# HagenMarin/SHAP-Transformer-ASR

Measured on NVIDIA B200. Metric: masked_coalition_forwards_per_sec, higher is better.
Workload: dtype bf16

## Files before the change

### include/w2s.h

```cpp
#ifndef W2S_H_
#define W2S_H_

#include <stdint.h>

#ifdef __cplusplus
extern "C" {
#endif

typedef struct w2s_handle w2s_handle;

#define W2S_MAX_CONV_LAYERS 8

enum {
  W2S_OUT_MAX     = 0,
  W2S_OUT_LOGIT   = 1,
  W2S_OUT_LOGPROB = 2,
  W2S_OUT_MEAN    = 3,
  W2S_OUT_LOGITS  = 4,
  W2S_OUT_CTC     = 5
};

enum {
  W2S_FLAG_VALIDATE_GEMM = 1,
  W2S_FLAG_VALIDATE_ATTN = 2,
// ... 63 lines not shown

int w2s_grad_waveforms(w2s_handle* h, const float* x_dev, int64_t n, int64_t L, int64_t ld,
                       const int32_t* frames_host, float* grad_dev, float* out_dev, void* stream);
int w2s_vjp_waveforms(w2s_handle* h, const float* x_dev, int64_t n, int64_t L, int64_t ld, const float* gout_dev,
                      float* grad_dev, float* out_dev, void* stream);
int w2s_grad_transcripts(w2s_handle* h, const float* x_dev, int64_t n, int64_t L, int64_t ld, const int32_t* which_host,
                         float* grad_dev, float* out_dev, void* stream);
int w2s_grad_debug(w2s_handle* h, int on);
int w2s_grad_rules(w2s_handle* h, int rules);
int64_t w2s_grad_peek(w2s_handle* h, const char* name, void* dst_dev, int64_t max_bytes, void* stream);

int w2s_mask(w2s_handle* h, const uint32_t* z_bits_dev, int64_t K, float* out_dev, void* stream);

int w2s_wls(w2s_handle* h, const uint32_t* z_bits_dev, const double* w_dev, const float* y_dev, int64_t K,
            int M, int D, const double* fx_dev, const double* fnull_dev, double* phi_dev, int32_t* status_dev,
            void* stream);

int64_t w2s_sample_rows(int M, int n_full, int n_paired, const int64_t* ind_set, int64_t n_ind,
                        int64_t samples_left, int64_t added, uint32_t* mt_key, int32_t* mt_pos,
                        uint32_t* z_words, double* weights, int64_t cap_rows, int64_t* ind_used);

int w2s_relative_buckets(int T, int num_buckets, int max_distance, int32_t* out);

int w2s_debug_gemm(int use_tcgen05, const void* a_bf16, const void* w_bf16, const float* bias,
                   const void* residual, int res_fp32, float alpha, void* out, int M, int N, int K, int act,
                   int out_fp32, void* stream);
int w2s_debug_attention(int use_tcgen05, const void* qkv, const void* pos_proj, int B, int T, int heads, float scale,
                        void* ctx, float* lse, void* stream);
int w2s_debug_attention_bias(int use_tcgen05, const void* qkv, const float* rel_bias, const float* gate, int B, int T,
                             int heads, float scale, void* ctx, float* lse, void* stream);
int w2s_debug_attention_bwd(int use_tcgen05, const void* qkv, const void* ctx, const void* dctx, const float* lse, int B,
                            int T, int heads, float scale, void* dqkv, void* stream);
int w2s_debug_ctc(const float* logits, int n, int T, int V, int ldl, const int32_t* labels_host, const int32_t* offsets_host,
                  int D, int blank, const int32_t* which_host, float* out_dev, float* dlogits_dev, void* stream);
int w2s_profile_enable(w2s_handle* h, int on);
int64_t w2s_profile_read(w2s_handle* h, char* names, int64_t names_cap, double* ms, double* flops, double* bytes,
                         int64_t* counts, int64_t max_entries);
int w2s_kernel_count(const w2s_handle* h, int64_t* launches_per_batch, int64_t* batch_tile);
int64_t w2s_launch_count(const w2s_handle* h);
double w2s_flops_per_forward(const w2s_handle* h, int64_t num_samples);

#ifdef __cplusplus
}
#endif
#endif
```

### shap_transformer_asr_b200/_lib.py

```python
from __future__ import annotations

import ctypes as C
import os

_HERE = os.path.dirname(os.path.abspath(__file__))
LIB_PATH = os.path.join(_HERE, "libw2s.so")

MAX_CONV_LAYERS = 8

OUT_MAX, OUT_LOGIT, OUT_LOGPROB, OUT_MEAN, OUT_LOGITS, OUT_CTC = 0, 1, 2, 3, 4, 5
MODE_IDS = {"max": OUT_MAX, "logit": OUT_LOGIT, "logprob": OUT_LOGPROB, "mean": OUT_MEAN, "logits": OUT_LOGITS}
FLAG_VALIDATE_GEMM, FLAG_VALIDATE_ATTN, FLAG_FP32_PRELN, FLAG_NO_GRAPH = 1, 2, 4, 16
MAX_BACKGROUND = 256
MAX_BANDS = 16
MAX_TRANSCRIPT = 512


class W2SConfig(C.Structure):
    _fields_ = [
        ("kind", C.c_int32),
        ("num_conv_layers", C.c_int32),
        ("conv_dim", C.c_int32 * MAX_CONV_LAYERS),
        ("conv_kernel", C.c_int32 * MAX_CONV_LAYERS),
        ("conv_stride", C.c_int32 * MAX_CONV_LAYERS),
# ... 35 lines not shown
    "w2s_set_transcripts": (C.c_int, [C.c_void_p, C.POINTER(C.c_int32), C.POINTER(C.c_int32), C.c_int, C.c_int,
                                      C.c_void_p]),
    "w2s_out_width": (C.c_int64, [C.c_void_p, C.c_int64]),
    "w2s_eval": (C.c_int, [C.c_void_p, C.c_void_p, C.c_int64, C.c_void_p, C.c_void_p]),
    "w2s_eval_waveforms": (C.c_int, [C.c_void_p, C.c_void_p, C.c_int64, C.c_int64, C.c_int64, C.c_void_p,
                                     C.c_void_p]),
    "w2s_grad_waveforms": (C.c_int, [C.c_void_p, C.c_void_p, C.c_int64, C.c_int64, C.c_int64, C.POINTER(C.c_int32),
                                     C.c_void_p, C.c_void_p, C.c_void_p]),
    "w2s_vjp_waveforms": (C.c_int, [C.c_void_p, C.c_void_p, C.c_int64, C.c_int64, C.c_int64, C.c_void_p, C.c_void_p,
                                    C.c_void_p, C.c_void_p]),
    "w2s_grad_transcripts": (C.c_int, [C.c_void_p, C.c_void_p, C.c_int64, C.c_int64, C.c_int64, C.POINTER(C.c_int32),
                                       C.c_void_p, C.c_void_p, C.c_void_p]),
    "w2s_grad_debug": (C.c_int, [C.c_void_p, C.c_int]),
    "w2s_grad_rules": (C.c_int, [C.c_void_p, C.c_int]),
    "w2s_grad_peek": (C.c_int64, [C.c_void_p, C.c_char_p, C.c_void_p, C.c_int64, C.c_void_p]),
    "w2s_mask": (C.c_int, [C.c_void_p, C.c_void_p, C.c_int64, C.c_void_p, C.c_void_p]),
    "w2s_wls": (C.c_int, [C.c_void_p, C.c_void_p, C.c_void_p, C.c_void_p, C.c_int64, C.c_int, C.c_int, C.c_void_p,
                          C.c_void_p, C.c_void_p, C.c_void_p, C.c_void_p]),
    "w2s_sample_rows": (C.c_int64, [C.c_int, C.c_int, C.c_int, C.c_void_p, C.c_int64, C.c_int64, C.c_int64, C.c_void_p,
                                    C.c_void_p, C.c_void_p, C.c_void_p, C.c_int64, C.c_void_p]),
    "w2s_relative_buckets": (C.c_int, [C.c_int, C.c_int, C.c_int, C.c_void_p]),
    "w2s_debug_gemm": (C.c_int, [C.c_int, C.c_void_p, C.c_void_p, C.c_void_p, C.c_void_p, C.c_int, C.c_float,
                                 C.c_void_p, C.c_int, C.c_int, C.c_int, C.c_int, C.c_int, C.c_void_p]),
    "w2s_debug_attention": (C.c_int, [C.c_int, C.c_void_p, C.c_void_p, C.c_int, C.c_int, C.c_int, C.c_float, C.c_void_p,
                                      C.c_void_p, C.c_void_p]),
    "w2s_debug_attention_bias": (C.c_int, [C.c_int, C.c_void_p, C.c_void_p, C.c_void_p, C.c_int, C.c_int, C.c_int, C.c_float,
                                           C.c_void_p, C.c_void_p, C.c_void_p]),
    "w2s_debug_attention_bwd": (C.c_int, [C.c_int, C.c_void_p, C.c_void_p, C.c_void_p, C.c_void_p, C.c_int, C.c_int, C.c_int,
                                          C.c_float, C.c_void_p, C.c_void_p]),
    "w2s_debug_ctc": (C.c_int, [C.c_void_p, C.c_int, C.c_int, C.c_int, C.c_int, C.POINTER(C.c_int32), C.POINTER(C.c_int32),
                                C.c_int, C.c_int, C.POINTER(C.c_int32), C.c_void_p, C.c_void_p, C.c_void_p]),
    "w2s_profile_enable": (C.c_int, [C.c_void_p, C.c_int]),
    "w2s_profile_read": (C.c_int64, [C.c_void_p, C.c_char_p, C.c_int64, C.POINTER(C.c_double), C.POINTER(C.c_double),
                                     C.POINTER(C.c_double), C.POINTER(C.c_int64), C.c_int64]),
    "w2s_kernel_count": (C.c_int, [C.c_void_p, C.POINTER(C.c_int64), C.POINTER(C.c_int64)]),
    "w2s_launch_count": (C.c_int64, [C.c_void_p]),
    "w2s_flops_per_forward": (C.c_double, [C.c_void_p, C.c_int64]),
}

_lib = None


def load():
    global _lib
    if _lib is not None:
        return _lib
# ... 12 lines not shown
```

### shap_transformer_asr_b200/csrc/api.cu

```cuda
#include "../../include/w2s.h"
#include "gemm.cuh"
#include "kernels.cuh"
#include "ctc.cuh"

#include <algorithm>
#include <cmath>
#include <cstdlib>
#include <cstring>
#include <functional>
#include <map>
#include <memory>
#include <string>
#include <vector>

using namespace w2s;
typedef __nv_bfloat16 bf16;

namespace {

thread_local std::string g_create_error;

struct LayerW {
  bf16 *wqkv = nullptr, *wo = nullptr, *w1 = nullptr, *w2 = nullptr;
  float *bqkv = nullptr, *bo = nullptr, *b1 = nullptr, *b2 = nullptr;
// ... 7 lines not shown
  float *gate_w = nullptr, *gate_b = nullptr, *gate_c = nullptr;
};

struct Step {
  std::string name;
  std::function<std::string(cudaStream_t)> run;
  double flops = 0.0;
  double bytes = 0.0;
};

struct ProfRec {
  std::string name;
  cudaEvent_t e0, e1;
  double flops, bytes;
};

struct Plan {
  int n = 0;
  std::vector<Step> steps;
  std::vector<GemmLaunch*> gemms;
  std::vector<AttnRelPlan*> attn_rel;
  std::vector<PosConvPlan*> posconv;
  std::vector<AttnFaPlan*> attn_fa;
  cudaGraphExec_t exec = nullptr;
  bool graph_failed = false;
  ~Plan() {
    if (exec) cudaGraphExecDestroy(exec);
    for (auto* f : attn_fa) attention_fa_free(f);
    for (auto* pc : posconv) posconv_free(pc);
    for (auto* g : gemms) delete g;
    for (auto* a : attn_rel) attention_rel_free(a);
  }
};

__global__ void set_dyn_kernel(DynArgs* dst, const DynArgs v) { *dst = v; }

struct GradW {
  bf16 *wqkvT = nullptr, *woT = nullptr, *w1T = nullptr, *w2T = nullptr;
  bf16 *f2w1T = nullptr, *f2w2T = nullptr, *pw1T = nullptr, *pw2T = nullptr, *wqkT = nullptr, *wvT = nullptr;
  float* dw_flip = nullptr;
  bf16 *pos_proj = nullptr, *pos_projT = nullptr;
};
struct GradPlan;

}

struct w2s_handle {
  w2s_config cfg{};
  int device = 0;
  int num_sms = 148;
  bool auto_batch = false;
// ... 355 lines not shown
  W2S_CUDA_OK(cudaDeviceSynchronize());
  return "";
}

GemmProblem plain_problem(const bf16* a, long long rows, int K, const bf16* w, int N) {
  GemmProblem p;
  p.a = a; p.a_cols = K; p.a_rows = rows; p.a_batches = 1; p.a_row_stride = K; p.a_batch_stride = rows * (long long)K;
  p.a_kb_per_row = K / 64; p.a_g_col = 0;
  p.w = w; p.M = (int)rows; p.N = N; p.K = K; p.Bz = 1; p.G = 1;
  p.epi.ldg = 0; p.epi.ldb = 0; p.epi.ldm = N;
  return p;
}

int64_t num_frames(const w2s_config& c, int64_t L, std::vector<int>* lens) {
  int64_t n = L;
  for (int l = 0; l < c.num_conv_layers; ++l) {
    if (n < c.conv_kernel[l]) return 0;
    n = (n - c.conv_kernel[l]) / c.conv_stride[l] + 1;
    if (lens) lens->push_back((int)n);
  }
  return n;
}

void free_workspace(w2s_handle* h) {
  h->plans.clear();
  for (void* p : h->ws_allocs) cudaFree(p);
  h->ws_allocs.clear();
  h->ws_L = -1;
}

std::string ensure_workspace(w2s_handle* h, long long L) {
  if (h->ws_L == L) return "";
  cudaDeviceSynchronize();
  free_workspace(h);
  const w2s_config& c = h->cfg;
  h->Tl.clear();
  const int64_t T = num_frames(c, L, &h->Tl);
  if (T <= 0) return "clip of " + std::to_string(L) + " samples is shorter than the conv receptive field";
  h->T = (int)T;
  h->Tp = (int)((T + 63) / 64 * 64);
  if (h->auto_batch) {
    long long k = 1;
    while ((long long)h->num_sms * 128 * k / T < 128) ++k;
    long long tile = (long long)h->num_sms * 128 * k / T;
    const long long conv0_bytes = (long long)h->Tl[0] * c.conv_dim[0] * 2;
    while (tile > 8 && tile * conv0_bytes > (8LL << 30)) tile /= 2;
    h->cfg.max_batch = (int)tile;
  }
  const size_t nb = (size_t)c.max_batch;
  const int H = c.hidden_size, I = c.intermediate_size;
  const int Cl = c.conv_dim[c.num_conv_layers - 1];
  auto& pool = h->ws_allocs;
  W2S_TRY(dalloc(pool, &h->gn_a, nb * c.conv_dim[0]));
  W2S_TRY(dalloc(pool, &h->gn_b, nb * c.conv_dim[0]));
  W2S_TRY(dalloc(pool, &h->gn_wb, nb * c.conv_dim[0] * 32));
  size_t szA = 0, szB = 0;
  for (int l = 0; l < c.num_conv_layers; ++l) {
    const size_t s = nb * (size_t)h->Tl[l] * c.conv_dim[l];
    if (l % 2 == 0) szA = s > szA ? s : szA;
    else szB = s > szB ? s : szB;
  }
  W2S_TRY(dalloc(pool, &h->bufA, szA));
  W2S_TRY(dalloc(pool, &h->bufB, szB ? szB : 1));
  const size_t rows = nb * (size_t)T;
  W2S_TRY(dalloc(pool, &h->fpn, rows * Cl));
  W2S_TRY(dalloc(pool, &h->h0, rows * H));
  W2S_TRY(dalloc(pool, &h->hb, rows * H));
  W2S_TRY(dalloc(pool, &h->h1, rows * H));
  W2S_TRY(dalloc(pool, &h->pre, rows * H));
  W2S_TRY(dalloc(pool, &h->qkv, rows * 4 * H));
  W2S_TRY(dalloc(pool, &h->ctx, rows * H));
  W2S_TRY(dalloc(pool, &h->ffn, rows * I));
  W2S_TRY(dalloc(pool, &h->logits, rows * (size_t)h->head_ldl));
  if (c.kind != 1) {
    W2S_TRY(dalloc(pool, &h->hp,
                   nb * (size_t)(T + c.num_conv_pos_embeddings) * c.num_conv_pos_embedding_groups * 64));
    if (c.kind == 2) {
      const int heads = c.num_attention_heads;
      std::vector<int32_t> bk((size_t)(2 * T - 1));
      if (w2s_relative_buckets((int)T, c.num_buckets, c.max_bucket_distance, bk.data()) != 0)
// ... 70 lines not shown
    const int T = h->T, H = c.hidden_size, V = c.vocab_size;
    HeadParams hp{};
    hp.h = h->hb; hp.w = h->head_w; hp.bias = h->head_b;
    hp.n = n; hp.T = T; hp.H = H; hp.V = V; hp.ldl = h->head_ldl; hp.dyn = h->dyn_dev;
    if (simt_gemm) {
      add("head", [=](cudaStream_t s) { return launch_head(hp, s); });
      return "";
    }
    GemmProblem p = plain(h->hb, (long long)n * T, H, h->head_w, h->head_ldl);
    p.epi.bias = h->head_b;
    p.epi.out = h->logits;
    p.epi.out_fp32 = 1;
    W2S_TRY(add_gemm("lm_head", p));
    const float* logits = h->logits;
    add("head_reduce", [=](cudaStream_t s) { return launch_head_reduce(logits, hp, s); }, 0.0,
        (double)n * T * V * 4.0);
    return "";
  }

  std::string build() {
    const w2s_config& c = h->cfg;
    const int T = h->T, H = c.hidden_size, I = c.intermediate_size;
    const bool layer = c.feat_extract_norm == 1;
    const long long rows = (long long)n * T;
    w2s_handle* hh = h;
    const int nn = n;

    {
      Conv0Params cp{};
      cp.dyn = h->dyn_dev;
      cp.n = n; cp.L = (int)h->ws_L; cp.T0 = h->Tl[0]; cp.C = c.conv_dim[0]; cp.kw = c.conv_kernel[0];
      cp.stride = c.conv_stride[0];
      cp.w = h->conv0_w; cp.bias = h->conv0_b; cp.gamma = h->norm0_g; cp.beta = h->norm0_b;
      cp.gn_a = h->gn_a; cp.gn_b = h->gn_b; cp.gn_wb = h->gn_wb;
      cp.ln_wbar = h->ln0_wbar; cp.ln_gram = h->ln0_gram; cp.ln_wb = h->ln0_wb;
      cp.ln_bmean = h->ln0_bmean; cp.ln_b2mean = h->ln0_b2mean; cp.ln_wb48 = h->ln0_wb48;
      cp.out = h->bufA;
      const int fill = this->fill;
      const double wave_bytes = (fill == FILL_BANDS ? 4.0 * h->bands_F : fill == FILL_BG ? 8.0 : 4.0) * (double)h->ws_L;
      if (!layer)
        add("conv0_stats", [=](cudaStream_t s) { return launch_conv0_stats(cp, s, fill); }, 0.0,
            (wave_bytes + (double)cp.C * (8.0 + 64.0)) * n);
      add("conv0", [=](cudaStream_t s) { return launch_conv0(cp, layer, s, fill); },
          2.0 * cp.T0 * (double)cp.C * cp.kw * n, ((double)cp.T0 * cp.C * 2.0 + wave_bytes) * n);
    }
    bf16* cur = h->bufA;
    for (int l = 1; l < c.num_conv_layers; ++l) {
      bf16* nxt = (l % 2 == 1) ? h->bufB : h->bufA;
      const int Cin = c.conv_dim[l - 1], Cout = c.conv_dim[l], kw = c.conv_kernel[l], st = c.conv_stride[l];
      const int Tin = h->Tl[l - 1], Tout = h->Tl[l];
      if ((st * Cin) % 64) return "conv layer " + std::to_string(l) + ": stride * in_channels must be a multiple of 64";
      GemmProblem p;
      p.a = cur; p.a_cols = (long long)st * Cin; p.a_rows = (Tin + st - 1) / st; p.a_batches = n;
      p.a_row_stride = (long long)st * Cin; p.a_batch_stride = (long long)Tin * Cin;
      p.a_kb_per_row = st * Cin / 64; p.a_g_col = 0;
      p.w = h->conv_w[l]; p.M = Tout; p.N = Cout; p.K = kw * Cin; p.Bz = n; p.G = 1;
      p.epi.bias = h->conv_b[l];
      p.epi.act = layer ? ACT_NONE : ACT_GELU;
      p.epi.out = nxt; p.epi.ldb = (long long)Tout * Cout; p.epi.ldm = Cout;
      W2S_TRY(add_gemm("conv" + std::to_string(l), p));
      if (layer)
        add_ln("conv" + std::to_string(l) + "_ln_gelu", nxt, 0, (long long)n * Tout, Cout, h->conv_ln_g[l],
               h->conv_ln_b[l], 1e-5f, ACT_GELU, nxt, nullptr);
      cur = nxt;
    }
    const int Cl = c.conv_dim[c.num_conv_layers - 1];
    add_ln("featproj_ln", cur, 0, rows, Cl, h->fp_ln_g, h->fp_ln_b, c.layer_norm_eps, ACT_NONE, h->fpn, nullptr);
    {
      GemmProblem p = plain(h->fpn, rows, Cl, h->fp_w, H);
      p.epi.bias = h->fp_b;
// ... 841 lines not shown
                             h->wls_work, (cudaStream_t)stream);
  return e.empty() ? 0 : fail(h, e);
}

int w2s_debug_gemm(int use_tcgen05, const void* a_bf16, const void* w_bf16, const float* bias, const void* residual,
                   int res_fp32, float alpha, void* out, int M, int N, int K, int act, int out_fp32, void* stream) {
  g_create_error.clear();
  std::string e = gemm_init();
  if (e.empty()) {
    GemmProblem p = PlanBuilder::plain((const bf16*)a_bf16, M, K, (const bf16*)w_bf16, N);
    p.epi.bias = bias; p.epi.act = act; p.epi.out = out; p.epi.out_fp32 = out_fp32;
    p.epi.residual = residual; p.epi.res_fp32 = res_fp32; p.epi.alpha = alpha;
    GemmLaunch gl;
    e = gemm_prepare(p, debug_num_sms(), &gl);
    if (e.empty()) e = use_tcgen05 ? gemm_launch_tc(gl, (cudaStream_t)stream) : gemm_launch_simt(gl, (cudaStream_t)stream);
  }
  if (!e.empty()) {
    g_create_error = e;
    return 1;
  }
  return 0;
}

int w2s_debug_attention(int use_tcgen05, const void* qkv, const void* pos_proj, int B, int T, int heads, float scale,
                        void* ctx, float* lse, void* stream) {
  g_create_error.clear();
  const cudaStream_t s = (cudaStream_t)stream;
  AttnParams ap = debug_attn_params(qkv, pos_proj, B, T, heads, scale);
  ap.ctx = (bf16*)ctx;
  ap.lse = lse;
  std::string e;
  if (B <= 0 || T <= 0 || heads <= 0 || !qkv || !ctx) {
    e = "debug_attention: need B, T', heads >= 1 and qkv / ctx buffers";
  } else if (lse && (pos_proj || !use_tcgen05)) {
    e = "debug_attention: only the tcgen05 kernel without relative positions writes the log-sum-exp";
  } else if (!(e = gemm_init()).empty()) {
  } else if (!use_tcgen05) {
    e = launch_attention_simt(ap, s);
  } else if (pos_proj) {
    AttnRelPlan* rp = nullptr;
    e = attention_rel_init();
    if (e.empty()) e = attention_rel_prepare(ap, &rp);
    if (e.empty()) e = attention_rel_launch(rp, s);
    if (rp) attention_rel_free(rp);
  } else {
    AttnFaPlan* fp = nullptr;
// ... 234 lines not shown
```

### shap_transformer_asr_b200/csrc/frontend.cu

```cuda
#include "kernels.cuh"

namespace w2s {

template <int FILL>
__global__ void __launch_bounds__(256) mask_kernel(const float* __restrict__ x, const uint16_t* __restrict__ seg_id,
                                                    const uint32_t* __restrict__ zbits, int zwords, long long L,
                                                    float baseline, float* __restrict__ out, long long ld,
                                                    const float* __restrict__ bg, int B, long long bg_ld, long long row0) {
  constexpr bool BG = FILL == FILL_BG;
  __shared__ uint32_t z[64];
  const long long g = BG ? row0 + blockIdx.y : blockIdx.y;
  const long long k = BG ? g / B : g;
  if (threadIdx.x < zwords) z[threadIdx.x] = zbits[k * zwords + threadIdx.x];
  __syncthreads();
  const long long i0 = ((long long)blockIdx.x * blockDim.x + threadIdx.x) * 4;
  if (i0 >= L) return;
  float* o = out + g * ld + i0;
  if constexpr (FILL == FILL_BANDS) {
    const int F = B;
    auto keep = [&](uint32_t sgm, int b) { const uint32_t c = sgm * F + b; return (z[c >> 5] >> (c & 31)) & 1u; };
    if (i0 + 4 <= L && ((ld & 3) == 0) && (bg_ld & 3) == 0) {
      const ushort4 sv = *reinterpret_cast<const ushort4*>(seg_id + i0);
      float4 r = make_float4(0.f, 0.f, 0.f, 0.f);
      for (int b = 0; b < F; ++b) {
// ... 53 lines not shown
  for (long long r0 = 0; r0 < rows; r0 += 65535) {
    const long long n = rows - r0 < 65535 ? rows - r0 : 65535;
    dim3 grid((unsigned)((L + 1023) / 1024), (unsigned)n);
    W2S_CUDA_OK(launch_pdl(mask_kernel<FILL_BG>, grid, dim3(256), 0, s, 1, x, seg_id, zbits, zwords, L, 0.f, out, ld, bg, B,
                           bg_ld, r0));
    W2S_CUDA_OK(cudaGetLastError());
  }
  return "";
}

std::string launch_mask_bands(const uint16_t* seg_id, const uint32_t* zbits, int zwords, long long K, long long L,
                              const float* comp, int F, long long comp_ld, float* out, long long ld, cudaStream_t s) {
  if (zwords > 64) return "mask: more than 2048 cells are not supported";
  for (long long k0 = 0; k0 < K; k0 += 65535) {
    const long long n = K - k0 < 65535 ? K - k0 : 65535;
    dim3 grid((unsigned)((L + 1023) / 1024), (unsigned)n);
    W2S_CUDA_OK(launch_pdl(mask_kernel<FILL_BANDS>, grid, dim3(256), 0, s, 1, (const float*)nullptr, seg_id,
                           zbits + k0 * zwords, zwords, L, 0.f, out + k0 * ld, ld, comp, F, comp_ld, 0LL));
    W2S_CUDA_OK(cudaGetLastError());
  }
  return "";
}

template <int FILL = FILL_PLAIN>
struct WaveRow {
  const float* x;
  const uint16_t* seg;
  const uint32_t* zs;
  float baseline;
  const float* fill;
  long long ld;
  int F;
  __device__ __forceinline__ float at(long long i) const {
    if constexpr (FILL == FILL_BANDS) {
      const uint32_t c0 = (uint32_t)__ldg(seg + i) * (uint32_t)F;
      float v = 0.f;
      for (int b = 0; b < F; ++b) {
        const uint32_t c = c0 + b;
        const float t = __ldg(x + b * ld + i);
        v += (zs[c >> 5] >> (c & 31)) & 1u ? t : 0.f;
      }
      return v;
    } else {
      const float v = __ldg(x + i);
      if constexpr (FILL == FILL_BG) {
        const uint32_t sgm = __ldg(seg + i);
        return (zs[sgm >> 5] >> (sgm & 31)) & 1u ? v : __ldg(fill + i);
      } else {
        if (!seg) return v;
        const uint32_t sgm = __ldg(seg + i);
        return (zs[sgm >> 5] >> (sgm & 31)) & 1u ? v : baseline;
      }
    }
  }
};
template <int FILL = FILL_PLAIN>
__device__ __forceinline__ WaveRow<FILL> wave_row(const DynArgs* __restrict__ dyn, int row, uint32_t* zs) {
  WaveRow<FILL> w;
  w.zs = zs;
  if constexpr (FILL == FILL_BG) {
    const long long g = dyn->row0 + row, B = dyn->B, k = g / B;
    const int zw = dyn->zwords;
    for (int i = threadIdx.x; i < zw; i += blockDim.x) zs[i] = dyn->zbits[k * zw + i];
    w.x = dyn->clip; w.seg = dyn->seg_id; w.baseline = 0.f;
    w.fill = dyn->bg + (g - k * B) * dyn->ld;
  } else if constexpr (FILL == FILL_BANDS) {
    const int zw = dyn->zwords;
    for (int i = threadIdx.x; i < zw; i += blockDim.x) zs[i] = dyn->zbits[(long long)row * zw + i];
    w.x = dyn->bands; w.seg = dyn->seg_id; w.ld = dyn->ld; w.F = dyn->F;
  } else if (dyn->clip) {
    const int zw = dyn->zwords;
    for (int i = threadIdx.x; i < zw; i += blockDim.x) zs[i] = dyn->zbits[(long long)row * zw + i];
    w.x = dyn->clip; w.seg = dyn->seg_id; w.baseline = dyn->baseline;
  } else {
    w.x = dyn->x + (long long)row * dyn->ld; w.seg = nullptr; w.baseline = 0.f;
  }
  __syncthreads();
  return w;
}

__device__ __forceinline__ double warp_sum_f64(double v) {
#pragma unroll
  for (int o = 16; o > 0; o >>= 1) v += __shfl_xor_sync(0xffffffffu, v, o);
  return v;
}

template <int KW, int FILL>
__global__ void __launch_bounds__(256, 1) conv0_stats_kernel(const Conv0Params p) {
  constexpr int NR = KW * (KW + 1) / 2;
  constexpr int NACC = KW + NR;
  __shared__ double red[8][NACC];
  __shared__ double tot[NACC];
  __shared__ uint32_t zs[64];
  const int row = blockIdx.x;
  const WaveRow<FILL> x = wave_row<FILL>(p.dyn, row, zs);
  double acc[NACC];
#pragma unroll
  for (int i = 0; i < NACC; ++i) acc[i] = 0.0;
  for (int t = threadIdx.x; t < p.T0; t += blockDim.x) {
    double xv[KW];
    const long long i0 = (long long)t * p.stride;
#pragma unroll
    for (int j = 0; j < KW; ++j) xv[j] = (double)x.at(i0 + j);
// ... 718 lines not shown
```

### shap_transformer_asr_b200/csrc/kernels.cuh

```cuda
#pragma once
#include "common.cuh"

namespace w2s {

std::string launch_mask(const float* x, const uint16_t* seg_id, const uint32_t* zbits, int zwords, long long K,
                        long long L, float baseline, float* out, long long ld, cudaStream_t s);
std::string launch_mask_bg(const float* x, const uint16_t* seg_id, const uint32_t* zbits, int zwords, long long K,
                           long long L, const float* bg, int B, long long bg_ld, float* out, long long ld, cudaStream_t s);
std::string launch_mask_bands(const uint16_t* seg_id, const uint32_t* zbits, int zwords, long long K, long long L,
                              const float* comp, int F, long long comp_ld, float* out, long long ld, cudaStream_t s);

enum Fill : int { FILL_PLAIN = 0, FILL_BG = 1, FILL_BANDS = 2 };

struct DynArgs {
  const float* x;
  long long ld;
  const float* clip;
  const uint16_t* seg_id;
  const uint32_t* zbits;
  int zwords;
  float baseline;
  float* out;
  int mode, D;
  const int* frames;
// ... 9 lines not shown
};

struct Conv0Params {
  const DynArgs* dyn;
  int n, L, T0, C, kw, stride;
  const float* w;
  const float* bias;
  const float* gamma;
  const float* beta;
  float* gn_a;
  float* gn_b;
  __nv_bfloat16* gn_wb;
  const float* ln_wbar;
  const float* ln_gram;
  const float* ln_wb;
  float ln_bmean, ln_b2mean;
  int pre_act;
  float* ln_rstd_out;
  const __nv_bfloat16* ln_wb48;
  __nv_bfloat16* out;
};
std::string launch_conv0_stats(const Conv0Params& p, cudaStream_t s, int fill = FILL_PLAIN);
std::string launch_conv0(const Conv0Params& p, bool layer_norm, cudaStream_t s, int fill = FILL_PLAIN);
std::string launch_conv0_ln_b(const float* w, const float* bias, const float* gamma, const float* beta, int C, int kw,
                              __nv_bfloat16* out, cudaStream_t s);
std::string launch_conv0_ln_prep(const float* w, const float* bias, int C, int kw, float* wbar, float* gram,
                                 float* wb, float* scalars , cudaStream_t s);

std::string launch_layernorm(const void* in, int in_fp32, long long rows, int H, const float* gamma,
                             const float* beta, float eps, int act, __nv_bfloat16* out, float* out_f32,
                             cudaStream_t s, const __nv_bfloat16* residual = nullptr);

std::string launch_pos_pad(const __nv_bfloat16* h, int B, int T, int H, int G, int kpos, __nv_bfloat16* out,
                           cudaStream_t s, int left = -1);

struct EpiParams;
struct PosConvPlan;
std::string posconv_init();
bool posconv_supported(int H, int G, int kpos);
std::string posconv_prepare(const __nv_bfloat16* x, const __nv_bfloat16* w, int B, int T, int H, int G, int kpos,
                            const EpiParams& epi, int num_sms, PosConvPlan** out);
std::string posconv_launch(const PosConvPlan* plan, cudaStream_t s);
void posconv_free(PosConvPlan* plan);

struct AttnParams {
  const __nv_bfloat16* qkv;
// ... 111 lines not shown
```

Baseline: 12500.

## Fuse conv0 and conv1 into one 2-SM tcgen05 kernel with on-chip conv0

Measured after the change: 12530 (median of 6 runs). About the same (+0.3%).

```diff
diff --git a/include/w2s.h b/include/w2s.h
--- a/include/w2s.h
+++ b/include/w2s.h
@@ -109,6 +109,8 @@
 
 int w2s_relative_buckets(int T, int num_buckets, int max_distance, int32_t* out);
 
+int w2s_debug_conv01(w2s_handle* h, const float* x_dev, int n, int64_t L, int64_t ld, int fused, void* out_dev,
+                     void* stream);
 int w2s_debug_gemm(int use_tcgen05, const void* a_bf16, const void* w_bf16, const float* bias,
                    const void* residual, int res_fp32, float alpha, void* out, int M, int N, int K, int act,
                    int out_fp32, void* stream);
diff --git a/shap_transformer_asr_b200/_lib.py b/shap_transformer_asr_b200/_lib.py
--- a/shap_transformer_asr_b200/_lib.py
+++ b/shap_transformer_asr_b200/_lib.py
@@ -81,6 +81,8 @@
     "w2s_relative_buckets": (C.c_int, [C.c_int, C.c_int, C.c_int, C.c_void_p]),
     "w2s_debug_gemm": (C.c_int, [C.c_int, C.c_void_p, C.c_void_p, C.c_void_p, C.c_void_p, C.c_int, C.c_float,
                                  C.c_void_p, C.c_int, C.c_int, C.c_int, C.c_int, C.c_int, C.c_void_p]),
+    "w2s_debug_conv01": (C.c_int, [C.c_void_p, C.c_void_p, C.c_int, C.c_int64, C.c_int64, C.c_int, C.c_void_p,
+                                   C.c_void_p]),
     "w2s_debug_attention": (C.c_int, [C.c_int, C.c_void_p, C.c_void_p, C.c_int, C.c_int, C.c_int, C.c_float, C.c_void_p,
                                       C.c_void_p, C.c_void_p]),
     "w2s_debug_attention_bias": (C.c_int, [C.c_int, C.c_void_p, C.c_void_p, C.c_void_p, C.c_int, C.c_int, C.c_int, C.c_float,
diff --git a/shap_transformer_asr_b200/csrc/api.cu b/shap_transformer_asr_b200/csrc/api.cu
--- a/shap_transformer_asr_b200/csrc/api.cu
+++ b/shap_transformer_asr_b200/csrc/api.cu
@@ -53,11 +53,13 @@
   std::vector<AttnRelPlan*> attn_rel;
   std::vector<PosConvPlan*> posconv;
   std::vector<AttnFaPlan*> attn_fa;
+  std::vector<Conv01Launch*> conv01;
   cudaGraphExec_t exec = nullptr;
   bool graph_failed = false;
   ~Plan() {
     if (exec) cudaGraphExecDestroy(exec);
     for (auto* f : attn_fa) attention_fa_free(f);
+    for (auto* f : conv01) conv01_free(f);
     for (auto* pc : posconv) posconv_free(pc);
     for (auto* g : gemms) delete g;
     for (auto* a : attn_rel) attention_rel_free(a);
@@ -459,6 +461,12 @@
   return n;
 }
 
+bool fused_conv01(const w2s_config& c) {
+  return c.feat_extract_norm != 1 && !(c.flags & W2S_FLAG_VALIDATE_GEMM) && c.num_conv_layers >= 2 &&
+         c.conv_dim[0] == 512 && c.conv_dim[1] == 512 && c.conv_kernel[0] == 10 && c.conv_stride[0] == 5 &&
+         c.conv_kernel[1] == 3 && c.conv_stride[1] == 2;
+}
+
 void free_workspace(w2s_handle* h) {
   h->plans.clear();
   for (void* p : h->ws_allocs) cudaFree(p);
@@ -492,7 +500,7 @@
   W2S_TRY(dalloc(pool, &h->gn_b, nb * c.conv_dim[0]));
   W2S_TRY(dalloc(pool, &h->gn_wb, nb * c.conv_dim[0] * 32));
   size_t szA = 0, szB = 0;
-  for (int l = 0; l < c.num_conv_layers; ++l) {
+  for (int l = fused_conv01(c) ? 1 : 0; l < c.num_conv_layers; ++l) {
     const size_t s = nb * (size_t)h->Tl[l] * c.conv_dim[l];
     if (l % 2 == 0) szA = s > szA ? s : szA;
     else szB = s > szB ? s : szB;
@@ -609,6 +617,7 @@
     const w2s_config& c = h->cfg;
     const int T = h->T, H = c.hidden_size, I = c.intermediate_size;
     const bool layer = c.feat_extract_norm == 1;
+    const bool fuse01 = fused_conv01(c);
     const long long rows = (long long)n * T;
     w2s_handle* hh = h;
     const int nn = n;
@@ -628,11 +637,23 @@
       if (!layer)
         add("conv0_stats", [=](cudaStream_t s) { return launch_conv0_stats(cp, s, fill); }, 0.0,
             (wave_bytes + (double)cp.C * (8.0 + 64.0)) * n);
-      add("conv0", [=](cudaStream_t s) { return launch_conv0(cp, layer, s, fill); },
-          2.0 * cp.T0 * (double)cp.C * cp.kw * n, ((double)cp.T0 * cp.C * 2.0 + wave_bytes) * n);
-    }
-    bf16* cur = h->bufA;
-    for (int l = 1; l < c.num_conv_layers; ++l) {
+      if (fuse01) {
+        Conv01Launch* cl = nullptr;
+        std::string err = conv01_prepare(h->dyn_dev, h->gn_wb, h->conv_w[1], h->conv_b[1], n, cp.T0, h->bufB,
+                                         h->num_sms, &cl);
+        if (cl) plan->conv01.push_back(cl);
+        W2S_TRY(err);
+        const int T1 = h->Tl[1];
+        add("conv0_conv1", [=](cudaStream_t s) { return conv01_launch(*cl, fill, s); },
+            (2.0 * T1 * 512.0 * 3.0 * 512.0 + 2.0 * cp.T0 * (double)cp.C * cp.kw) * n,
+            ((double)T1 * 512.0 * 2.0 + wave_bytes) * n);
+      } else {
+        add("conv0", [=](cudaStream_t s) { return launch_conv0(cp, layer, s, fill); },
+            2.0 * cp.T0 * (double)cp.C * cp.kw * n, ((double)cp.T0 * cp.C * 2.0 + wave_bytes) * n);
+      }
+    }
+    bf16* cur = fuse01 ? h->bufB : h->bufA;
+    for (int l = fuse01 ? 2 : 1; l < c.num_conv_layers; ++l) {
       bf16* nxt = (l % 2 == 1) ? h->bufB : h->bufA;
       const int Cin = c.conv_dim[l - 1], Cout = c.conv_dim[l], kw = c.conv_kernel[l], st = c.conv_stride[l];
       const int Tin = h->Tl[l - 1], Tout = h->Tl[l];
@@ -1520,6 +1541,76 @@
   return 0;
 }
 
+namespace {
+std::string debug_conv01(w2s_handle* h, const float* x, int n, long long L, long long ld, int fused, void* out,
+                         cudaStream_t s) {
+  const w2s_config& c = h->cfg;
+  w2s_config shapes = c;
+  shapes.flags &= ~W2S_FLAG_VALIDATE_GEMM;
+  if (!fused_conv01(shapes)) return "w2s_debug_conv01: the model's conv0 / conv1 are not of the fused kind";
+  if (n <= 0 || L < 13 || ld < L || !x || !out) return "w2s_debug_conv01: bad arguments";
+  W2S_TRY(gemm_init());
+  const int C = 512, T0 = (int)((L - 10) / 5 + 1), T1 = (T0 - 3) / 2 + 1;
+  std::vector<void*> tmp;
+  auto alloc = [&](void** p, size_t bytes) -> std::string {
+    W2S_CUDA_OK(cudaMalloc(p, bytes));
+    tmp.push_back(*p);
+    return "";
+  };
+  std::string e = [&]() -> std::string {
+    DynArgs* dyn = nullptr;
+    float *gn_a = nullptr, *gn_b = nullptr;
+    bf16 *gn_wb = nullptr, *y0 = nullptr;
+    W2S_TRY(alloc((void**)&dyn, sizeof(DynArgs)));
+    W2S_TRY(alloc((void**)&gn_a, sizeof(float) * n * C));
+    W2S_TRY(alloc((void**)&gn_b, sizeof(float) * n * C));
+    W2S_TRY(alloc((void**)&gn_wb, sizeof(bf16) * n * C * 32));
+    DynArgs d{};
+    d.x = x;
+    d.ld = ld;
+    W2S_CUDA_OK(cudaMemcpyAsync(dyn, &d, sizeof(d), cudaMemcpyHostToDevice, s));
+    Conv0Params cp{};
+    cp.dyn = dyn;
+    cp.n = n; cp.L = (int)L; cp.T0 = T0; cp.C = C; cp.kw = 10; cp.stride = 5;
+    cp.w = h->conv0_w; cp.bias = h->conv0_b; cp.gamma = h->norm0_g; cp.beta = h->norm0_b;
+    cp.gn_a = gn_a; cp.gn_b = gn_b; cp.gn_wb = gn_wb;
+    W2S_TRY(launch_conv0_stats(cp, s, FILL_PLAIN));
+    if (fused) {
+      Conv01Launch* cl = nullptr;
+      std::string err = conv01_prepare(dyn, gn_wb, h->conv_w[1], h->conv_b[1], n, T0, (bf16*)out, h->num_sms, &cl);
+      if (err.empty()) err = conv01_launch(*cl, FILL_PLAIN, s);
+      if (cl) conv01_free(cl);
+      return err;
+    }
+    W2S_TRY(alloc((void**)&y0, sizeof(bf16) * (size_t)n * T0 * C));
+    cp.out = y0;
+    W2S_TRY(launch_conv0(cp, false, s, FILL_PLAIN));
+    GemmProblem p;
+    p.a = y0; p.a_cols = 2 * C; p.a_rows = (T0 + 1) / 2; p.a_batches = n;
+    p.a_row_stride = 2 * C; p.a_batch_stride = (long long)T0 * C;
+    p.a_kb_per_row = 2 * C / 64; p.a_g_col = 0;
+    p.w = h->conv_w[1]; p.M = T1; p.N = C; p.K = 3 * C; p.Bz = n; p.G = 1;
+    p.epi.bias = h->conv_b[1];
+    p.epi.act = ACT_GELU;
+    p.epi.out = out; p.epi.ldb = (long long)T1 * C; p.epi.ldm = C;
+    GemmLaunch gl;
+    W2S_TRY(gemm_prepare(p, h->num_sms, &gl));
+    return gemm_launch_tc(gl, s);
+  }();
+  const cudaError_t se = cudaStreamSynchronize(s);
+  for (void* p : tmp) cudaFree(p);
+  if (e.empty() && se != cudaSuccess) e = std::string("w2s_debug_conv01: ") + cudaGetErrorString(se);
+  return e;
+}
+}
+
+int w2s_debug_conv01(w2s_handle* h, const float* x_dev, int n, int64_t L, int64_t ld, int fused, void* out_dev,
+                     void* stream) {
+  if (!h) return 1;
+  const std::string e = debug_conv01(h, x_dev, n, L, ld, fused, out_dev, (cudaStream_t)stream);
+  return e.empty() ? 0 : fail(h, e);
+}
+
 int w2s_debug_attention(int use_tcgen05, const void* qkv, const void* pos_proj, int B, int T, int heads, float scale,
                         void* ctx, float* lse, void* stream) {
   g_create_error.clear();
diff --git a/shap_transformer_asr_b200/csrc/conv01.cu b/shap_transformer_asr_b200/csrc/conv01.cu
--- /dev/null
+++ b/shap_transformer_asr_b200/csrc/conv01.cu
@@ -0,0 +1,411 @@
+#include "gemm.cuh"
+#include "gemm_epi.cuh"
+#include "wave_row.cuh"
+
+#include <mutex>
+
+namespace w2s {
+
+namespace {
+
+constexpr int kC = 512;
+constexpr int kStride0 = 5, kKw0 = 10;
+constexpr int kFrames = 257;
+constexpr int kRows = 272;
+constexpr int kLda = 80;
+constexpr int kSamples = (kFrames - 1) * kStride0 + kKw0;
+constexpr int kBStages = 3;
+constexpr int kBHalf = 128 * 128;
+constexpr int kBBytes = 2 * kBHalf;
+constexpr int kEBytes = 17 * 1024;
+constexpr int kOBytes = 16 * 1024;
+constexpr int kAStages = 2;
+constexpr int kABytes = kEBytes + kOBytes;
+constexpr int kOffA = kBStages * kBBytes;
+constexpr int kOffEpi = kOffA + kAStages * kABytes;
+constexpr int kOffI = kOffEpi + 8 * 4096;
+constexpr int kOffX = kOffI + kRows * kLda;
+constexpr int kOffBias = kOffX + ((kSamples * 4 + 15) & ~15);
+constexpr int kOffZ = kOffBias + kC * 4;
+constexpr int kOffBar = kOffZ + 64 * 4;
+constexpr size_t kSmem = (size_t)kOffBar + 128 + 1024;
+static_assert(kOffA % 1024 == 0 && kABytes % 1024 == 0 && kOffEpi % 1024 == 0, "swizzled tiles need 1024-byte alignment");
+static_assert(kSmem <= 227 * 1024, "shared memory");
+
+constexpr int kProducers = 12;
+constexpr int kThreads = (8 + kProducers + 3) * 32;
+constexpr int kWarpTma = 8 + kProducers, kWarpMma = kWarpTma + 1, kWarpAlloc = kWarpTma + 2;
+
+__device__ __forceinline__ void producer_sync() { asm volatile("bar.sync 1, %0;" ::"n"(kProducers * 32) : "memory"); }
+__device__ __forceinline__ void mbar_arrive_remote(uint32_t cluster_addr) {
+  asm volatile("mbarrier.arrive.release.cluster.shared::cluster.b64 _, [%0];" ::"r"(cluster_addr) : "memory");
+}
+__device__ __forceinline__ uint32_t bf16_bits(float v) { return (uint32_t)__bfloat16_as_ushort(__float2bfloat16_rn(v)); }
+
+}
+
+struct Conv01Dev {
+  const DynArgs* dyn;
+  const __nv_bfloat16* gn_wb;
+  const float* bias;
+  int T0, T1, units_m, num_units;
+};
+
+template <int FILL>
+__global__ void __launch_bounds__(kThreads, 1)
+conv01_kernel(const __grid_constant__ CUtensorMap mapW, const __grid_constant__ CUtensorMap mapOut, const Conv01Dev p) {
+  const uint32_t rank = cluster_ctarank();
+  const bool leader = rank == 0;
+  const int unit0 = (int)(blockIdx.x >> 1), unit_step = (int)(gridDim.x >> 1);
+  extern __shared__ uint8_t smem_raw[];
+  const uint32_t raw = smem_u32(smem_raw);
+  const uint32_t base = (raw + 1023u) & ~1023u;
+  uint8_t* base_ptr = smem_raw + (base - raw);
+  const uint32_t sB = base, sA = base + kOffA, sEpi = base + kOffEpi, sI = base + kOffI;
+  float* xs = reinterpret_cast<float*>(base_ptr + kOffX);
+  float* sbias = reinterpret_cast<float*>(base_ptr + kOffBias);
+  uint32_t* zs = reinterpret_cast<uint32_t*>(base_ptr + kOffZ);
+  const uint32_t bars = base + kOffBar;
+  auto bfull = [&](int s) { return bars + 8u * s; };
+  auto bempty = [&](int s) { return bars + 8u * (kBStages + s); };
+  auto afull = [&](int s) { return bars + 8u * (2 * kBStages + s); };
+  auto aempty = [&](int s) { return bars + 8u * (2 * kBStages + kAStages + s); };
+  const uint32_t tfull = bars + 8u * (2 * kBStages + 2 * kAStages);
+  auto tempty = [&](int h) { return bars + 8u * (2 * kBStages + 2 * kAStages + 1 + h); };
+  const uint32_t tmem_slot = bars + 8u * (2 * kBStages + 2 * kAStages + 3);
+  volatile uint32_t* tmem_slot_ptr =
+      reinterpret_cast<volatile uint32_t*>(base_ptr + kOffBar + 8 * (2 * kBStages + 2 * kAStages + 3));
+
+  const int warp = threadIdx.x >> 5, lane = threadIdx.x & 31;
+  if (warp == kWarpTma && lane == 0) {
+    tma_prefetch_desc(&mapW);
+    tma_prefetch_desc(&mapOut);
+  }
+  if (warp == kWarpMma && lane == 0) {
+    for (int s = 0; s < kBStages; ++s) {
+      mbar_init(bfull(s), 1);
+      mbar_init(bempty(s), 1);
+    }
+    for (int s = 0; s < kAStages; ++s) {
+      mbar_init(afull(s), 2 * kProducers);
+      mbar_init(aempty(s), 1);
+    }
+    mbar_init(tfull, 1);
+    for (int h = 0; h < 2; ++h) mbar_init(tempty(h), 16);
+    fence_barrier_init();
+    fence_proxy_async();
+  }
+  if (warp == kWarpAlloc) {
+    tmem_alloc_2sm<512>(tmem_slot);
+    tmem_relinquish_2sm();
+  }
+  if (warp < 8 && p.bias)
+    for (int i = threadIdx.x; i < kC; i += 256) sbias[i] = __ldg(p.bias + i);
+  tc_fence_before();
+  __syncthreads();
+  cluster_sync_all();
+  tc_fence_after();
+  const uint32_t tmem_base = *tmem_slot_ptr;
+
+  if (warp == kWarpTma) {
+    if (elect_one()) {
+      int stage = 0;
+      uint32_t phase = 0;
+      for (int unit = unit0; unit < p.num_units; unit += unit_step) {
+        for (int cb = 0; cb < kC / 64; ++cb) {
+          for (int tap = 0; tap < 3; ++tap) {
+            mbar_wait(bempty(stage), phase ^ 1u);
+            const uint32_t full_leader = mapa_u32(bfull(stage), 0);
+            if (leader) mbar_expect_tx(bfull(stage), 2 * kBBytes);
+            const uint32_t dst = sB + stage * kBBytes;
+#pragma unroll
+            for (int h = 0; h < 2; ++h)
+              tma_load_3d_2sm(dst + h * kBHalf, &mapW, full_leader, tap * kC + cb * 64, h * 256 + (int)rank * 128, 0);
+            if (++stage == kBStages) {
+              stage = 0;
+              phase ^= 1u;
+            }
+          }
+        }
+      }
+    }
+  } else if (warp == kWarpMma) {
+    if (leader && elect_one()) {
+      constexpr uint32_t idesc = umma_idesc_bf16(256, 256);
+      int bs = 0, as = 0;
+      uint32_t bph = 0, aph = 0, tph = 0;
+      for (int unit = unit0; unit < p.num_units; unit += unit_step) {
+        for (int cb = 0; cb < kC / 64; ++cb) {
+          mbar_wait(afull(as), aph);
+          tc_fence_after();
+          const uint32_t ae = sA + as * kABytes;
+          for (int tap = 0; tap < 3; ++tap) {
+            mbar_wait(bfull(bs), bph);
+            tc_fence_after();
+            const uint64_t da = umma_desc_sw128(tap == 0 ? ae : tap == 1 ? ae + kEBytes : ae + 128u);
+            const uint32_t sb = sB + bs * kBBytes;
+#pragma unroll
+            for (int h = 0; h < 2; ++h) {
+              if (cb == 0 && tap == 0) {
+                mbar_wait(tempty(h), tph ^ 1u);
+                tc_fence_after();
+              }
+              const uint64_t db = umma_desc_sw128(sb + h * kBHalf);
+#pragma unroll
+              for (int k = 0; k < 4; ++k)
+                umma_bf16_2sm(tmem_base + h * 256, da + 2u * k, db + 2u * k, idesc, (cb | tap | k) != 0 ? 1u : 0u);
+            }
+            umma_commit_2sm_mc(bempty(bs), (uint16_t)0x3);
+            if (++bs == kBStages) {
+              bs = 0;
+              bph ^= 1u;
+            }
+          }
+          umma_commit_2sm_mc(aempty(as), (uint16_t)0x3);
+          if (++as == kAStages) {
+            as = 0;
+            aph ^= 1u;
+          }
+        }
+        umma_commit_2sm_mc(tfull, (uint16_t)0x3);
+        tph ^= 1u;
+      }
+    }
+  } else if (warp >= 8 && warp < 8 + kProducers) {
+    const int pw = warp - 8, ptid = (int)threadIdx.x - 256, hh = pw & 1;
+    static_assert(kProducers % 2 == 0, "a producer warp keeps one channel half");
+    const int g = lane >> 2, t = lane & 3;
+    const uint32_t a_lane = sI + (lane & 15) * kLda + (lane >> 4) * 16;
+    const long long lim = (long long)(p.T0 - 1) * kStride0 + kKw0;
+    int as = 0;
+    uint32_t aph = 0;
+    for (int unit = unit0; unit < p.num_units; unit += unit_step) {
+      const int b = unit / p.units_m, mu = unit - b * p.units_m;
+      const int f0 = 2 * (2 * mu + (int)rank) * 128;
+      producer_sync();
+      const WaveRow<FILL> x = wave_row_load<FILL>(p.dyn, b, zs, ptid, kProducers * 32);
+      producer_sync();
+      {
+        const long long s0 = (long long)f0 * kStride0;
+        constexpr int kPer = (kSamples + kProducers * 32 - 1) / (kProducers * 32);
+        float sv[kPer];
+#pragma unroll
+        for (int k = 0; k < kPer; ++k) {
+          const int i = ptid + kProducers * 32 * k;
+          sv[k] = (i < kSamples && s0 + i < lim) ? x.at(s0 + i) : 0.f;
+        }
+#pragma unroll
+        for (int k = 0; k < kPer; ++k)
+          if (ptid + kProducers * 32 * k < kSamples) xs[ptid + kProducers * 32 * k] = sv[k];
+      }
+      producer_sync();
+      for (int r = ptid; r < kRows; r += kProducers * 32) {
+        uint32_t w[16];
+        if (r < kFrames && f0 + r < p.T0) {
+          uint32_t hi[kKw0], lo[kKw0];
+#pragma unroll
+          for (int j = 0; j < kKw0; ++j) {
+            const float v = xs[r * kStride0 + j];
+            const __nv_bfloat16 h = __float2bfloat16_rn(v);
+            hi[j] = (uint32_t)__bfloat16_as_ushort(h);
+            lo[j] = bf16_bits(v - __bfloat162float(h));
+          }
+#pragma unroll
+          for (int k = 0; k < 15; ++k) {
+            auto e = [&](int i) { return i < kKw0 ? hi[i] : i < 2 * kKw0 ? lo[i - kKw0] : hi[i - 2 * kKw0]; };
+            w[k] = e(2 * k) | (e(2 * k + 1) << 16);
+          }
+          w[15] = 0x3f803f80u;
+        } else {
+#pragma unroll
+          for (int k = 0; k < 16; ++k) w[k] = 0u;
+        }
+#pragma unroll
+        for (int q = 0; q < 4; ++q) sts128(sI + r * kLda + q * 16, w[4 * q], w[4 * q + 1], w[4 * q + 2], w[4 * q + 3]);
+      }
+      producer_sync();
+
+      const uint32_t* wb = reinterpret_cast<const uint32_t*>(p.gn_wb + (long long)b * kC * 32);
+#pragma unroll 1
+      for (int cb = 0; cb < kC / 64; ++cb) {
+        uint32_t bfrag[4][2][2];
+#pragma unroll
+        for (int nt = 0; nt < 4; ++nt) {
+          const int ch = cb * 64 + hh * 32 + (g >> 1) * 8 + nt * 2 + (g & 1);
+#pragma unroll
+          for (int ks = 0; ks < 2; ++ks) {
+            bfrag[nt][ks][0] = __ldg(wb + ch * 16 + 8 * ks + t);
+            bfrag[nt][ks][1] = __ldg(wb + ch * 16 + 8 * ks + t + 4);
+          }
+        }
+        mbar_wait(aempty(as), aph ^ 1u);
+        const uint32_t ae = sA + as * kABytes, ao = ae + kEBytes;
+#pragma unroll 1
+        for (int mb = pw >> 1; mb < kRows / 16; mb += kProducers / 2) {
+          uint32_t a[2][4];
+          ldmatrix_x4(a[0], a_lane + mb * 16 * kLda);
+          ldmatrix_x4(a[1], a_lane + mb * 16 * kLda + 32);
+          float c[4][4];
+#pragma unroll
+          for (int nt = 0; nt < 4; ++nt) {
+            c[nt][0] = c[nt][1] = c[nt][2] = c[nt][3] = 0.f;
+            mma_bf16_16816(c[nt], a[0], bfrag[nt][0]);
+            mma_bf16_16816(c[nt], a[1], bfrag[nt][1]);
+          }
+#pragma unroll
+          for (int r = 0; r < 2; ++r) {
+            const int i = mb * 16 + g + 8 * r;
+            if (i < kFrames) {
+              const uint32_t wr = (uint32_t)(i >> 1);
+              uint32_t pk[4];
+#pragma unroll
+              for (int q = 0; q < 4; ++q) {
+                const float2 y = gelu_erf2(make_float2(c[q][2 * r], c[q][2 * r + 1]));
+                pk[q] = pack_bf16x2(y.x, y.y);
+              }
+              sts128(((g & 1) ? ao : ae) + wr * 128u + ((((uint32_t)(hh * 4 + t)) ^ (wr & 7u)) << 4), pk[0], pk[1], pk[2],
+                     pk[3]);
+            }
+          }
+        }
+        fence_proxy_async();
+        __syncwarp();
+        if (lane == 0) {
+          if (leader) mbar_arrive(afull(as));
+          else mbar_arrive_remote(mapa_u32(afull(as), 0));
+        }
+        if (++as == kAStages) {
+          as = 0;
+          aph ^= 1u;
+        }
+      }
+    }
+  } else if (warp < 8) {
+    const int q = warp & 3, hsel = warp >> 2;
+    const bool lead = elect_one();
+    const uint32_t stg = sEpi + warp * 4096;
+    const uint32_t stg_row = stg + lane * 128;
+    EpiParams e;
+    e.act = ACT_GELU;
+    uint32_t tph = 0;
+    for (int unit = unit0; unit < p.num_units; unit += unit_step) {
+      const int b = unit / p.units_m, mu = unit - b * p.units_m;
+      const int m0 = (2 * mu + (int)rank) * 128;
+      const int m = m0 + q * 32 + lane;
+      mbar_wait(tfull, tph);
+      tc_fence_after();
+#pragma unroll 1
+      for (int h = 0; h < 2; ++h) {
+        const uint32_t t0 = tmem_base + (static_cast<uint32_t>(q * 32) << 16) + h * 256;
+        auto sub_col = [&](int sidx) { return (2 * (sidx >> 1) + hsel) * 64 + (sidx & 1) * 32; };
+        float v[32];
+        tmem_ld_32x32_issue(t0 + sub_col(0), v);
+#pragma unroll 1
+        for (int sidx = 0; sidx < 4; ++sidx) {
+          const int c = sub_col(sidx);
+          const int sub = sidx & 1;
+          tmem_ld_wait();
+          epi_math32(e, p.bias ? sbias + h * 256 + c : nullptr, kC, 0, b, m, h * 256 + c, m < p.T1, v);
+          uint32_t pk[16];
+#pragma unroll
+          for (int j = 0; j < 16; ++j) pk[j] = pack_bf16x2(v[2 * j], v[2 * j + 1]);
+          if (sidx + 1 < 4) tmem_ld_32x32_issue(t0 + sub_col(sidx + 1), v);
+          if (sub == 0) {
+            if (lead) tma_store_wait_read();
+            __syncwarp();
+          }
+#pragma unroll
+          for (int j = 0; j < 4; ++j)
+            sts128(stg_row + (((uint32_t)(sub * 4 + j) ^ ((uint32_t)lane & 7u)) << 4), pk[4 * j], pk[4 * j + 1],
+                   pk[4 * j + 2], pk[4 * j + 3]);
+          if (sub == 1) {
+            fence_proxy_async();
+            __syncwarp();
+            if (lead) {
+              tma_store_4d(&mapOut, stg, h * 256 + c - 32, m0 + q * 32, b, 0);
+              tma_store_commit();
+            }
+          }
+        }
+        tc_fence_before();
+        __syncwarp();
+        if (lane == 0) {
+          if (leader) mbar_arrive(tempty(h));
+          else mbar_arrive_cluster(mapa_u32(tempty(h), 0));
+        }
+      }
+      tph ^= 1u;
+    }
+    if (lead) tma_store_wait_all();
+  }
+
+  tc_fence_before();
+  __syncthreads();
+  cluster_sync_all();
+  if (warp == kWarpAlloc) {
+    tc_fence_after();
+    tmem_dealloc_2sm<512>(tmem_base);
+  }
+}
+
+struct Conv01Launch {
+  CUtensorMap mapW, mapOut;
+  Conv01Dev dev;
+  int grid = 0;
+};
+
+static std::once_flag g_conv01_once;
+static std::string g_conv01_err;
+
+std::string conv01_prepare(const DynArgs* dyn, const __nv_bfloat16* gn_wb, const __nv_bfloat16* w1, const float* b1,
+                           int n, int T0, __nv_bfloat16* out, int num_sms, Conv01Launch** out_launch) {
+  W2S_TRY(gemm_init());
+  std::call_once(g_conv01_once, [] {
+    cudaError_t e = cudaFuncSetAttribute(conv01_kernel<FILL_PLAIN>, cudaFuncAttributeMaxDynamicSharedMemorySize, (int)kSmem);
+    if (e == cudaSuccess)
+      e = cudaFuncSetAttribute(conv01_kernel<FILL_BG>, cudaFuncAttributeMaxDynamicSharedMemorySize, (int)kSmem);
+    if (e == cudaSuccess)
+      e = cudaFuncSetAttribute(conv01_kernel<FILL_BANDS>, cudaFuncAttributeMaxDynamicSharedMemorySize, (int)kSmem);
+    if (e != cudaSuccess) g_conv01_err = std::string("cudaFuncSetAttribute(conv01_kernel): ") + cudaGetErrorString(e);
+  });
+  W2S_TRY(g_conv01_err);
+  if (T0 < 3) return "conv0_conv1: fewer than 3 conv0 frames";
+  auto* l = new Conv01Launch();
+  *out_launch = l;
+  const int T1 = (T0 - 3) / 2 + 1;
+  l->dev.dyn = dyn; l->dev.gn_wb = gn_wb; l->dev.bias = b1;
+  l->dev.T0 = T0; l->dev.T1 = T1;
+  l->dev.units_m = (T1 + 255) / 256;
+  l->dev.num_units = l->dev.units_m * n;
+  const int clusters = l->dev.num_units < num_sms / 2 ? l->dev.num_units : num_sms / 2;
+  l->grid = 2 * clusters;
+  {
+    uint64_t dims[3] = {3 * kC, kC, 1};
+    uint64_t str[2] = {3 * kC * 2, 3ull * kC * kC * 2};
+    uint32_t box[3] = {64, 128, 1};
+    W2S_TRY(make_tensor_map_bf16(&l->mapW, w1, 3, dims, str, box));
+  }
+  {
+    uint64_t dims[4] = {kC, (uint64_t)T1, (uint64_t)n, 1};
+    uint64_t str[3] = {kC * 2, (uint64_t)T1 * kC * 2, (uint64_t)n * T1 * kC * 2};
+    uint32_t box[4] = {64, 32, 1, 1};
+    W2S_TRY(make_tensor_map_bf16(&l->mapOut, out, 4, dims, str, box));
+  }
+  return "";
+}
+
+void conv01_free(Conv01Launch* l) { delete l; }
+
+std::string conv01_launch(const Conv01Launch& l, int fill, cudaStream_t s) {
+  if (l.grid == 0) return "";
+  if (fill == FILL_BANDS)
+    W2S_CUDA_OK(launch_pdl(conv01_kernel<FILL_BANDS>, dim3(l.grid), dim3(kThreads), kSmem, s, 2, l.mapW, l.mapOut, l.dev));
+  else if (fill == FILL_BG)
+    W2S_CUDA_OK(launch_pdl(conv01_kernel<FILL_BG>, dim3(l.grid), dim3(kThreads), kSmem, s, 2, l.mapW, l.mapOut, l.dev));
+  else
+    W2S_CUDA_OK(launch_pdl(conv01_kernel<FILL_PLAIN>, dim3(l.grid), dim3(kThreads), kSmem, s, 2, l.mapW, l.mapOut, l.dev));
+  W2S_CUDA_OK(cudaGetLastError());
+  return "";
+}
+
+}
diff --git a/shap_transformer_asr_b200/csrc/frontend.cu b/shap_transformer_asr_b200/csrc/frontend.cu
--- a/shap_transformer_asr_b200/csrc/frontend.cu
+++ b/shap_transformer_asr_b200/csrc/frontend.cu
@@ -1,4 +1,5 @@
 #include "kernels.cuh"
+#include "wave_row.cuh"
 
 namespace w2s {
 
@@ -99,63 +100,6 @@
   return "";
 }
 
-template <int FILL = FILL_PLAIN>
-struct WaveRow {
-  const float* x;
-  const uint16_t* seg;
-  const uint32_t* zs;
-  float baseline;
-  const float* fill;
-  long long ld;
-  int F;
-  __device__ __forceinline__ float at(long long i) const {
-    if constexpr (FILL == FILL_BANDS) {
-      const uint32_t c0 = (uint32_t)__ldg(seg + i) * (uint32_t)F;
-      float v = 0.f;
-      for (int b = 0; b < F; ++b) {
-        const uint32_t c = c0 + b;
-        const float t = __ldg(x + b * ld + i);
-        v += (zs[c >> 5] >> (c & 31)) & 1u ? t : 0.f;
-      }
-      return v;
-    } else {
-      const float v = __ldg(x + i);
-      if constexpr (FILL == FILL_BG) {
-        const uint32_t sgm = __ldg(seg + i);
-        return (zs[sgm >> 5] >> (sgm & 31)) & 1u ? v : __ldg(fill + i);
-      } else {
-        if (!seg) return v;
-        const uint32_t sgm = __ldg(seg + i);
-        return (zs[sgm >> 5] >> (sgm & 31)) & 1u ? v : baseline;
-      }
-    }
-  }
-};
-template <int FILL = FILL_PLAIN>
-__device__ __forceinline__ WaveRow<FILL> wave_row(const DynArgs* __restrict__ dyn, int row, uint32_t* zs) {
-  WaveRow<FILL> w;
-  w.zs = zs;
-  if constexpr (FILL == FILL_BG) {
-    const long long g = dyn->row0 + row, B = dyn->B, k = g / B;
-    const int zw = dyn->zwords;
-    for (int i = threadIdx.x; i < zw; i += blockDim.x) zs[i] = dyn->zbits[k * zw + i];
-    w.x = dyn->clip; w.seg = dyn->seg_id; w.baseline = 0.f;
-    w.fill = dyn->bg + (g - k * B) * dyn->ld;
-  } else if constexpr (FILL == FILL_BANDS) {
-    const int zw = dyn->zwords;
-    for (int i = threadIdx.x; i < zw; i += blockDim.x) zs[i] = dyn->zbits[(long long)row * zw + i];
-    w.x = dyn->bands; w.seg = dyn->seg_id; w.ld = dyn->ld; w.F = dyn->F;
-  } else if (dyn->clip) {
-    const int zw = dyn->zwords;
-    for (int i = threadIdx.x; i < zw; i += blockDim.x) zs[i] = dyn->zbits[(long long)row * zw + i];
-    w.x = dyn->clip; w.seg = dyn->seg_id; w.baseline = dyn->baseline;
-  } else {
-    w.x = dyn->x + (long long)row * dyn->ld; w.seg = nullptr; w.baseline = 0.f;
-  }
-  __syncthreads();
-  return w;
-}
-
 __device__ __forceinline__ double warp_sum_f64(double v) {
 #pragma unroll
   for (int o = 16; o > 0; o >>= 1) v += __shfl_xor_sync(0xffffffffu, v, o);
diff --git a/shap_transformer_asr_b200/csrc/kernels.cuh b/shap_transformer_asr_b200/csrc/kernels.cuh
--- a/shap_transformer_asr_b200/csrc/kernels.cuh
+++ b/shap_transformer_asr_b200/csrc/kernels.cuh
@@ -55,6 +55,11 @@
 };
 std::string launch_conv0_stats(const Conv0Params& p, cudaStream_t s, int fill = FILL_PLAIN);
 std::string launch_conv0(const Conv0Params& p, bool layer_norm, cudaStream_t s, int fill = FILL_PLAIN);
+struct Conv01Launch;
+std::string conv01_prepare(const DynArgs* dyn, const __nv_bfloat16* gn_wb, const __nv_bfloat16* w1, const float* b1,
+                           int n, int T0, __nv_bfloat16* out, int num_sms, Conv01Launch** out_launch);
+std::string conv01_launch(const Conv01Launch& l, int fill, cudaStream_t s);
+void conv01_free(Conv01Launch* l);
 std::string launch_conv0_ln_b(const float* w, const float* bias, const float* gamma, const float* beta, int C, int kw,
                               __nv_bfloat16* out, cudaStream_t s);
 std::string launch_conv0_ln_prep(const float* w, const float* bias, int C, int kw, float* wbar, float* gram,
diff --git a/shap_transformer_asr_b200/csrc/wave_row.cuh b/shap_transformer_asr_b200/csrc/wave_row.cuh
--- /dev/null
+++ b/shap_transformer_asr_b200/csrc/wave_row.cuh
@@ -0,0 +1,85 @@
+#pragma once
+#include "kernels.cuh"
+
+namespace w2s {
+
+template <int FILL = FILL_PLAIN>
+struct WaveRow {
+  const float* x;
+  const uint16_t* seg;
+  const uint32_t* zs;
+  float baseline;
+  const float* fill;
+  long long ld;
+  int F;
+  __device__ __forceinline__ float at(long long i) const {
+    if constexpr (FILL == FILL_BANDS) {
+      const uint32_t c0 = (uint32_t)__ldg(seg + i) * (uint32_t)F;
+      float v = 0.f;
+      for (int b = 0; b < F; ++b) {
+        const uint32_t c = c0 + b;
+        const float t = __ldg(x + b * ld + i);
+        v += (zs[c >> 5] >> (c & 31)) & 1u ? t : 0.f;
+      }
+      return v;
+    } else {
+      const float v = __ldg(x + i);
+      if constexpr (FILL == FILL_BG) {
+        const uint32_t sgm = __ldg(seg + i);
+        return (zs[sgm >> 5] >> (sgm & 31)) & 1u ? v : __ldg(fill + i);
+      } else {
+        if (!seg) return v;
+        const uint32_t sgm = __ldg(seg + i);
+        return (zs[sgm >> 5] >> (sgm & 31)) & 1u ? v : baseline;
+      }
+    }
+  }
+};
+template <int FILL = FILL_PLAIN>
+__device__ __forceinline__ WaveRow<FILL> wave_row(const DynArgs* __restrict__ dyn, int row, uint32_t* zs) {
+  WaveRow<FILL> w;
+  w.zs = zs;
+  if constexpr (FILL == FILL_BG) {
+    const long long g = dyn->row0 + row, B = dyn->B, k = g / B;
+    const int zw = dyn->zwords;
+    for (int i = threadIdx.x; i < zw; i += blockDim.x) zs[i] = dyn->zbits[k * zw + i];
+    w.x = dyn->clip; w.seg = dyn->seg_id; w.baseline = 0.f;
+    w.fill = dyn->bg + (g - k * B) * dyn->ld;
+  } else if constexpr (FILL == FILL_BANDS) {
+    const int zw = dyn->zwords;
+    for (int i = threadIdx.x; i < zw; i += blockDim.x) zs[i] = dyn->zbits[(long long)row * zw + i];
+    w.x = dyn->bands; w.seg = dyn->seg_id; w.ld = dyn->ld; w.F = dyn->F;
+  } else if (dyn->clip) {
+    const int zw = dyn->zwords;
+    for (int i = threadIdx.x; i < zw; i += blockDim.x) zs[i] = dyn->zbits[(long long)row * zw + i];
+    w.x = dyn->clip; w.seg = dyn->seg_id; w.baseline = dyn->baseline;
+  } else {
+    w.x = dyn->x + (long long)row * dyn->ld; w.seg = nullptr; w.baseline = 0.f;
+  }
+  __syncthreads();
+  return w;
+}
+template <int FILL>
+__device__ __forceinline__ WaveRow<FILL> wave_row_load(const DynArgs* __restrict__ dyn, int row, uint32_t* zs, int tid,
+                                                       int nthreads) {
+  WaveRow<FILL> w;
+  w.zs = zs;
+  const int zw = dyn->zwords;
+  if constexpr (FILL == FILL_BG) {
+    const long long g = dyn->row0 + row, B = dyn->B, k = g / B;
+    for (int i = tid; i < zw; i += nthreads) zs[i] = dyn->zbits[k * zw + i];
+    w.x = dyn->clip; w.seg = dyn->seg_id; w.baseline = 0.f;
+    w.fill = dyn->bg + (g - k * B) * dyn->ld;
+  } else if constexpr (FILL == FILL_BANDS) {
+    for (int i = tid; i < zw; i += nthreads) zs[i] = dyn->zbits[(long long)row * zw + i];
+    w.x = dyn->bands; w.seg = dyn->seg_id; w.ld = dyn->ld; w.F = dyn->F;
+  } else if (dyn->clip) {
+    for (int i = tid; i < zw; i += nthreads) zs[i] = dyn->zbits[(long long)row * zw + i];
+    w.x = dyn->clip; w.seg = dyn->seg_id; w.baseline = dyn->baseline;
+  } else {
+    w.x = dyn->x + (long long)row * dyn->ld; w.seg = nullptr; w.baseline = 0.f;
+  }
+  return w;
+}
+
+}
```
